# LuoweiZhou/VLP

Measured on AMD Instinct MI355X. Metric: samples/sec/node (COCO 100-region, seq64, bs64xN) fp16, higher is better.
Workload: dtype f16; 1 GPU; COCO Captions fine-tune shape: BERT-base 12L, 100 regions x 2048-d, seq_len 64 (L=167), bs 64/GPU, fwd+bwd+FP16 FusedAdam, dropout 0.1, dynamic loss scale; global_batch=64, parallelism=dp1, batch_pool=8, skipped_steps=0, rccl_ranks=1, optimizer=replicated, first_leg_packed=False

## Files before the change

### include/vlp_hip.h

```cpp
#ifndef VLP_HIP_H
#define VLP_HIP_H

#include <stdint.h>

#ifdef __cplusplus
extern "C" {
#endif

#define VLP_ABI_VERSION 5

typedef enum {
    VLP_OK = 0,
    VLP_ERR_BAD_ARG = -1,
    VLP_ERR_HIP = -2,
    VLP_ERR_WORKSPACE = -3
} vlp_status;

enum { VLP_ACT_NONE = 0, VLP_ACT_GELU = 1, VLP_ACT_RELU = 2, VLP_ACT_TANH = 3,
       VLP_ACT_GELU_SAVE_GRAD = 4  };
enum { VLP_MUL_NONE = 0, VLP_MUL_GELU_GRAD = 1, VLP_MUL_RELU_MASK = 2, VLP_MUL_PLAIN = 3  };

int vlp_version(void);
const char* vlp_last_error_string(void);
int vlp_lab_build(void);
// ... 93 lines not shown
} vlp_attn_bwd_args;
int vlp_attn_bwd(const vlp_attn_bwd_args* a, void* stream);

int vlp_mask_pack(const int64_t* mask, uint8_t* out, uint8_t* out_t, int32_t B, int32_t L, int32_t Lp, void* stream);

typedef struct {
    const void* x; int64_t ldx;
    const void* gamma; const void* beta;
    void* y; int64_t ldy;
    float* mean; float* rstd;
    int32_t M, H; float eps;
    float dropout_p; uint64_t seed; uint32_t rng_stream;
    const int32_t* row_map;
} vlp_layernorm_fwd_args;
int vlp_layernorm_fwd(const vlp_layernorm_fwd_args* a, void* stream);

typedef struct {
    const void* dy; int64_t lddy;
    const void* x; int64_t ldx;
    const void* gamma;
    const float* mean; const float* rstd;
    void* dx; int64_t lddx;
    void* dx_drop; int64_t lddxd;
    void* dgamma; void* dbeta;
    int32_t M, H; int32_t beta;
    float dy_drop_p; uint64_t dy_seed; uint32_t dy_stream;
    float out_drop_p; uint64_t out_seed; uint32_t out_stream;
    void* workspace; int64_t workspace_bytes;
    int32_t defer_reduce;
    const int32_t* row_map;
// ... 354 lines not shown
```

### vlp_amd/_lib.py

```python
import ctypes as C
import os

import torch

_HERE = os.path.dirname(os.path.abspath(__file__))
LIB_PATH = os.environ.get("VLP_HIP_LIB") or os.path.join(_HERE, "libvlp_hip.so")

ACT_NONE, ACT_GELU, ACT_RELU, ACT_TANH, ACT_GELU_SAVE_GRAD = 0, 1, 2, 3, 4
MUL_NONE, MUL_GELU_GRAD, MUL_RELU_MASK, MUL_PLAIN = 0, 1, 2, 3
ROWS_X, ROWS_MUL, ROWS_RES, ROWS_Y = 1, 2, 4, 8

vp, i64, i32, f32, u64, u32 = C.c_void_p, C.c_int64, C.c_int32, C.c_float, C.c_uint64, C.c_uint32


class GemmNtArgs(C.Structure):
    _fields_ = [("X", vp), ("ldx", i64), ("W", vp), ("ldw", i64), ("Y", vp), ("ldy", i64), ("bias", vp),
                ("residual", vp), ("ldr", i64), ("preact", vp), ("ldp", i64), ("mul_src", vp), ("ldm", i64),
                ("M", i32), ("N", i32), ("K", i32), ("act", i32), ("mul_mode", i32), ("alpha", f32),
                ("dropout_p", f32), ("seed", u64), ("rng_stream", u32), ("variant", i32), ("row_map", vp)]


class GemmTnArgs(C.Structure):
    _fields_ = [("A", vp), ("lda", i64), ("B", vp), ("ldb", i64), ("C", vp), ("ldc", i64),
                ("M", i32), ("N", i32), ("K", i32), ("beta", i32), ("workspace", vp), ("workspace_bytes", i64),
# ... 197 lines not shown
    "vlp_logsoftmax_topk": (C.c_int, [vp, i64, i32, i32, i32, vp, i32, i32, vp, vp, vp]),
    "vlp_beam_select": (C.c_int, [C.POINTER(BeamSelectArgs), vp]),
    "vlp_ngram_candidates": (C.c_int, [vp, vp, i32, i32, i32, i32, vp, i32, vp, i64, vp, vp]),
    "vlp_logsoftmax_topk_list": (C.c_int, [vp, i64, i32, i32, i32, vp, i64, vp, i32, i32, vp, vp, vp]),
    "vlp_kv_gather": (C.c_int, [vp, i64, vp, i64, vp, i32, i32, i32, i32, vp]),
    "vlp_embed_bwd_workspace_floats": (C.c_int64, [i32, i32, i32, i32]),
    "vlp_mask_build": (C.c_int, [vp, vp, vp, vp, vp, i32, i32, i32, vp, i32, vp]),
    "vlp_vis_pe_prep": (C.c_int, [C.POINTER(VisPePrepArgs), vp]),
    "vlp_sample_rows": (C.c_int, [vp, i64, i32, i32, C.c_uint64, C.c_uint32, vp, i64, vp, i64, vp]),
    "vlp_sample_rows_rep": (C.c_int, [vp, i64, i32, i32, i32, vp, C.c_uint64, C.c_uint32, vp, i64, vp, i64, vp, i64, vp]),
    "vlp_sample_rows_filtered": (C.c_int, [vp, i64, i32, i32, i32, vp, C.c_uint64, C.c_uint32, C.c_float, i32, C.c_float, vp, i64, vp, i64, vp, i64,
                                           vp, vp, vp]),
    "vlp_argmax_rows": (C.c_int, [vp, i64, i32, i32, vp, i64, vp, i64, vp]),
    "vlp_mask_pack": (C.c_int, [vp, vp, vp, i32, i32, i32, vp]),
    "vlp_layernorm_fwd": (C.c_int, [C.POINTER(LayerNormFwdArgs), vp]),
    "vlp_layernorm_bwd_workspace_bytes": (i64, [i32]),
    "vlp_layernorm_bwd": (C.c_int, [C.POINTER(LayerNormBwdArgs), vp]),
    "vlp_layernorm_bwd_rows": (C.c_int, [C.POINTER(LayerNormBwdArgs), vp, i32, i32, vp]),
    "vlp_layernorm_bwd_reduce_batched": (C.c_int, [vp, vp, i32, i32, i32, i32, vp]),
    "vlp_embed_fwd": (C.c_int, [C.POINTER(EmbedFwdArgs), vp]),
    "vlp_embed_bwd": (C.c_int, [C.POINTER(EmbedBwdArgs), vp]),
    "vlp_embed_bwd_pos": (C.c_int, [C.POINTER(EmbedBwdPosArgs), vp]),
    "vlp_scst_layout": (C.c_int, [C.POINTER(ScstLayoutArgs), vp]),
    "vlp_token_logprob_fwd": (C.c_int, [C.POINTER(TokenLogprobFwdArgs), vp]),
    "vlp_token_logprob_bwd": (C.c_int, [C.POINTER(TokenLogprobBwdArgs), vp]),
    "vlp_token_policy_fwd": (C.c_int, [C.POINTER(TokenPolicyFwdArgs), vp]),
    "vlp_token_policy_bwd": (C.c_int, [C.POINTER(TokenPolicyBwdArgs), vp]),
    "vlp_region_mask_build": (C.c_int, [vp, i32, i32, i32, vp, vp]),
    "vlp_pretext_fwd": (C.c_int, [C.POINTER(PretextFwdArgs), vp]),
    "vlp_pretext_bwd": (C.c_int, [C.POINTER(PretextBwdArgs), vp]),
# ... 138 lines not shown
                      ptr(preact), (ldp if ldp is not None else (preact.stride(0) if preact is not None else 0)),
                      ptr(mul_src), (ldm if ldm is not None else (mul_src.stride(0) if mul_src is not None else 0)),
                      M, N, K, act, mul_mode, alpha, dropout_p, seed, rng_stream, variant, ptr(row_map))


def gemm_nt(x, w, y, M, N, K, ldx=None, ldw=None, ldy=None, bias=None, residual=None, ldr=None, preact=None, ldp=None,
            mul_src=None, ldm=None, act=ACT_NONE, mul_mode=MUL_NONE, alpha=1.0, dropout_p=0.0, seed=0, rng_stream=0,
            variant=0, row_map=None):
    _req_cuda(x, w, y, row_map)
    a = _gemm_nt_args(x, w, y, M, N, K, ldx, ldw, ldy, bias, residual, ldr, preact, ldp, mul_src, ldm, act, mul_mode, alpha, dropout_p, seed,
                      rng_stream, variant, row_map)
    _check(load().vlp_gemm_nt(C.byref(a), stream_ptr()))


def gemm_nt_rows(x, w, y, live, flags, M, N, K, ldx=None, ldw=None, ldy=None, bias=None, residual=None, ldr=None, mul_src=None, ldm=None,
                 mul_mode=MUL_NONE, alpha=1.0, dropout_p=0.0, seed=0, rng_stream=0, variant=0, row_map=None):
    _req_cuda(x, w, y, live, row_map)
    a = _gemm_nt_args(x, w, y, M, N, K, ldx, ldw, ldy, bias, residual, ldr, None, None, mul_src, ldm, ACT_NONE, mul_mode, alpha, dropout_p, seed,
                      rng_stream, variant, row_map)
    _check(load().vlp_gemm_nt_rows(C.byref(a), ptr(live), flags, stream_ptr()))


def gemm_nt_resolved_variant():
    return int(load().vlp_gemm_nt_resolved_variant())


def gemm_nt_splitk_workspace_bytes(M, N, splits):
    return int(load().vlp_gemm_nt_splitk_workspace_bytes(M, N, splits))


def gemm_nt_splitk(x, w, y, M, N, K, splits, workspace, ldx=None, ldw=None, ldy=None, bias=None, residual=None, ldr=None, preact=None, ldp=None,
                   mul_src=None, ldm=None, act=ACT_NONE, mul_mode=MUL_NONE, alpha=1.0, dropout_p=0.0, seed=0, rng_stream=0):
    _req_cuda(x, w, y, workspace)
# ... 200 lines not shown
    _check(load().vlp_sample_rows_filtered(ptr(logits), ld, rows, V, rep, ptr(seed_cell), int(seed_add) & 0xFFFFFFFFFFFFFFFF, rng_stream,
                                           float(temperature), int(top_k), float(top_p), ptr(ids), ids.stride(0), ptr(ids2),
                                           ids2.stride(0) if ids2 is not None else 0, ptr(logp), logp.stride(0), ptr(cutoff), ptr(kept), stream_ptr()))


def mask_pack(mask_i64, out_u8, B, L, Lp, out_t=None):
    _req_cuda(mask_i64, out_u8, out_t)
    _check(load().vlp_mask_pack(ptr(mask_i64), ptr(out_u8), ptr(out_t), B, L, Lp, stream_ptr()))


def layernorm_fwd(x, gamma, beta, y, M, H, mean=None, rstd=None, eps=1e-5, dropout_p=0.0, seed=0, rng_stream=0, ldx=None, ldy=None, row_map=None):
    _req_cuda(x, gamma, beta, y, row_map)
    a = LayerNormFwdArgs(ptr(x), ldx if ldx is not None else x.stride(0), ptr(gamma), ptr(beta), ptr(y),
                         ldy if ldy is not None else y.stride(0), ptr(mean), ptr(rstd), M, H, eps, dropout_p, seed, rng_stream, ptr(row_map))
    _check(load().vlp_layernorm_fwd(C.byref(a), stream_ptr()))


def layernorm_bwd_workspace_bytes(H):
    return int(load().vlp_layernorm_bwd_workspace_bytes(H))


def layernorm_bwd(dy, x, gamma, mean, rstd, dx, dgamma, dbeta, M, H, workspace, beta=0, dx_drop=None,
                  dy_drop=(0.0, 0, 0), out_drop=(0.0, 0, 0), defer_reduce=False, row_map=None):
    _req_cuda(dy, x, gamma, mean, rstd, dx, dgamma, dbeta, workspace, row_map)
    a = LayerNormBwdArgs(ptr(dy), dy.stride(0), ptr(x), x.stride(0), ptr(gamma), ptr(mean), ptr(rstd), ptr(dx), dx.stride(0),
                         ptr(dx_drop), dx_drop.stride(0) if dx_drop is not None else 0, ptr(dgamma), ptr(dbeta), M, H, beta,
                         dy_drop[0], dy_drop[1], dy_drop[2], out_drop[0], out_drop[1], out_drop[2],
                         ptr(workspace), _nbytes(workspace), 1 if defer_reduce else 0, ptr(row_map))
    _check(load().vlp_layernorm_bwd(C.byref(a), stream_ptr()))

# ... 411 lines not shown
```

### vlp_amd/csrc/gemm_nt.hip

```cpp
#include "common.h"
#include "gemm_nt.h"
#include "gemm_nt_epilogue.h"

#define BM 128
#define BK 64


#ifdef VLP_NT_DEBUG
__device__ unsigned long long g_nt_trace[4096 * 4];
#define NT_TRACE(slot) do { if (wid == 0 && lane == 0 && blockIdx.x < 4096) g_nt_trace[blockIdx.x * 4 + (slot)] = wall_clock64(); } while (0)
extern "C" int vlp_debug_read_nt_trace(void* dst, int64_t bytes) { return (int)hipMemcpyFromSymbol(dst, HIP_SYMBOL(g_nt_trace), bytes); }
#else
#define NT_TRACE(slot) do { } while (0)
#endif
DEVFN int swz_x(int r) { return r & 7; }
DEVFN int swz_w(int r) { return (((r >> 4) & 3) << 1) | ((r >> 1) & 1); }

template <int VARIANT, int BM_T, int BN_T, bool SG, int NSR, int EPI, bool ROWS>
DEVFN void gemm_nt_body(const GemmNtParams& p, const int32_t* __restrict__ live, int live_flags) {
    extern __shared__ __attribute__((aligned(16))) char smem_raw[];
    f16* smem = reinterpret_cast<f16*>(smem_raw);
    constexpr int WN_ = BN_T / 64;
    constexpr int T = (BM_T / 64) * WN_ * 64;
    constexpr int RPP = T / 8;
// ... 295 lines not shown
#pragma unroll
        for (int h = 0; h < 2; ++h)
            nt_epilogue8<SG>(p, m, ncol0 + 8 * h, v + 8 * h, rkey, true);
    }
#ifdef VLP_NT_DEBUG
    NT_TRACE(2);
    asm volatile("s_waitcnt vmcnt(0)" ::: "memory");
    NT_TRACE(3);
#endif
}

template <int VARIANT, int BM_T, int BN_T, bool SG, int NSR = 0, int EPI = 0>
__global__ __launch_bounds__((BM_T / 64) * (BN_T / 64) * 64, (VARIANT == 3 ? (BN_T == 256 ? 4 : BM_T / 128) : ((VARIANT == 2 || BN_T == 256) ? 4 : 2))) void gemm_nt_kernel(GemmNtParams p) {
    gemm_nt_body<VARIANT, BM_T, BN_T, SG, NSR, EPI, false>(p, nullptr, 0);
}
__global__ __launch_bounds__(256, 1) void gemm_nt_rows_kernel(GemmNtParams p, const int32_t* __restrict__ live, int live_flags) {
    gemm_nt_body<3, 128, 128, false, 0, 0, true>(p, live, live_flags);
}

int vlp_gemm_nt_fill_params(const vlp_gemm_nt_args* a, GemmNtParams& p) {
    VLP_CHECK_ARG(a != nullptr, "vlp_gemm_nt: null args");
    VLP_CHECK_ARG(a->X && a->W && a->Y, "vlp_gemm_nt: null operand");
    VLP_CHECK_ARG(a->M > 0 && a->N > 0 && a->K > 0, "vlp_gemm_nt: bad shape M=%d N=%d K=%d", a->M, a->N, a->K);
    VLP_CHECK_ARG(a->K % BK == 0, "vlp_gemm_nt: K=%d must be a multiple of %d (pad with vlp_copy2d)", a->K, BK);
    VLP_CHECK_ARG(a->ldx % 8 == 0 && a->ldw % 8 == 0 && a->ldy % 8 == 0, "vlp_gemm_nt: leading dims must be multiples of 8 halfs");
    VLP_CHECK_ARG(a->ldx >= a->K && a->ldw >= a->K, "vlp_gemm_nt: ldx/ldw < K");
    const int n8 = (a->N + 7) / 8 * 8;
    VLP_CHECK_ARG(a->ldy >= n8, "vlp_gemm_nt: ldy=%lld < roundup8(N)=%d", (long long)a->ldy, n8);
    VLP_CHECK_ARG(((uintptr_t)a->X | (uintptr_t)a->W | (uintptr_t)a->Y) % 16 == 0, "vlp_gemm_nt: operands must be 16-byte aligned");
    if (a->residual) VLP_CHECK_ARG(a->ldr % 8 == 0 && a->ldr >= n8 && (uintptr_t)a->residual % 16 == 0, "vlp_gemm_nt: bad residual layout");
    if (a->preact) VLP_CHECK_ARG(a->ldp % 8 == 0 && a->ldp >= n8 && (uintptr_t)a->preact % 16 == 0, "vlp_gemm_nt: bad preact layout");
    if (a->mul_mode != VLP_MUL_NONE)
// ... 115 lines not shown
    }
#undef LAUNCH_RING
#undef LAUNCH_NT
#undef LAUNCH_NT_
    VLP_CHECK_LAUNCH("vlp_gemm_nt");
    return VLP_OK;
}

extern "C" int vlp_gemm_nt_rows(const vlp_gemm_nt_args* a, const int32_t* live, int32_t flags, void* stream) {
    VLP_ENTER(a ? a->X : nullptr, "vlp_gemm_nt_rows");
    GemmNtParams p;
    const int frc = vlp_gemm_nt_fill_params(a, p);
    if (frc != VLP_OK) return frc;
    VLP_CHECK_ARG(live != nullptr, "vlp_gemm_nt_rows: null row list");
    VLP_CHECK_ARG((flags & ~(VLP_ROWS_X | VLP_ROWS_MUL | VLP_ROWS_RES | VLP_ROWS_Y)) == 0, "vlp_gemm_nt_rows: bad flags %d", flags);
    VLP_CHECK_ARG(!a->preact && nt_epilogue_is_light(p) && a->act != VLP_ACT_GELU_SAVE_GRAD,
                  "vlp_gemm_nt_rows: the listed-row form carries the dgrad epilogues (bias, stored multiplier, dropout, residual) only");
    p.xcd_remap = (a->variant & 8) ? 1 : 0;
    t_last_variant = 17 | (a->variant & 8);
    const size_t smem = (size_t)4 * (128 + 128) * BK * sizeof(f16);
    VLP_ONCE_PER_DEVICE((void)hipFuncSetAttribute((const void*)gemm_nt_rows_kernel, hipFuncAttributeMaxDynamicSharedMemorySize, (int)smem));
    p.tiles_n = cdiv(a->N, 128);
    hipLaunchKernelGGL(gemm_nt_rows_kernel, dim3(cdiv(a->M, 128) * p.tiles_n), dim3(256), smem, (hipStream_t)stream, p, live, (int)flags);
    VLP_CHECK_LAUNCH("vlp_gemm_nt_rows");
    return VLP_OK;
}

extern "C" int vlp_gemm_nt_splitk(const vlp_gemm_nt_args* a, int32_t splits, void* workspace, int64_t workspace_bytes, void* stream) {
    VLP_ENTER(a ? a->X : nullptr, "vlp_gemm_nt_splitk");
    GemmNtParams p;
    const int frc = vlp_gemm_nt_fill_params(a, p);
    if (frc != VLP_OK) return frc;
    VLP_CHECK_ARG(a->act != VLP_ACT_GELU_SAVE_GRAD, "vlp_gemm_nt_splitk: VLP_ACT_GELU_SAVE_GRAD is not provided (training-shape kernels only)");
    return vlp_gemm_nt_splitk_launch(p, splits, (float*)workspace, workspace_bytes, (hipStream_t)stream);
}
```

### vlp_amd/csrc/layernorm.hip

```cpp
#include "common.h"
#include <climits>
#include <cstdlib>

#define LN_THREADS 256
#define LN_WAVES 4

DEVFN uint32_t ln_fwd_rowkey(const DropCtx& drop, const int32_t* __restrict__ row_map, int row) {
    return drop.thresh ? drop_rowkey(drop, row_map ? (uint64_t)(uint32_t)row_map[row] : (uint64_t)row) : 0u;
}
DEVFN f16 ln_fwd_out(float v, float mu, float rs, f16 gamma, f16 beta, float m) { return (f16)(((float)gamma * ((v - mu) * rs) + (float)beta) * m); }

template <int NP>
__global__ __launch_bounds__(LN_THREADS) void layernorm_fwd_kernel(
    const f16* __restrict__ x, int64_t ldx, const f16* __restrict__ gamma, const f16* __restrict__ beta,
    f16* __restrict__ y, int64_t ldy, float* __restrict__ mean, float* __restrict__ rstd, int M, int H, float eps, DropCtx drop, const int32_t* __restrict__ row_map) {
    const int lane = threadIdx.x & 63;
    const int wave = blockIdx.x * LN_WAVES + (threadIdx.x >> 6);
    const int nwaves = gridDim.x * LN_WAVES;
    const float invH = 1.f / (float)H;
    for (int row = wave; row < M; row += nwaves) {
        const f16* xr = x + (int64_t)row * ldx;
        float v[NP][4];
        float s = 0.f;
#pragma unroll
        for (int k = 0; k < NP; ++k) {
            const int c = 256 * k + 4 * lane;
            if (c < H) {
                f16x4 t = ld4(xr + c);
#pragma unroll
                for (int e = 0; e < 4; ++e) { v[k][e] = (float)t[e]; s += v[k][e]; }
            } else {
#pragma unroll
                for (int e = 0; e < 4; ++e) v[k][e] = 0.f;
            }
        }
// ... 16 lines not shown
#pragma unroll
        for (int k = 0; k < NP; ++k) {
            const int c = 256 * k + 4 * lane;
            if (c < H) {
                f16x4 gv = ld4(gamma + c), bv = ld4(beta + c), o;
                float m4[4] = {1.f, 1.f, 1.f, 1.f};
                if (drop.thresh) drop_mult4(drop, rkey, (uint32_t)c, m4);
#pragma unroll
                for (int e = 0; e < 4; ++e) o[e] = ln_fwd_out(v[k][e], mu, rs, gv[e], bv[e], m4[e]);
                st4_out<VLP_SS_LN>(yr + c, o);
            }
        }
    }
}

template <int NC>
__global__ __launch_bounds__(LN_THREADS, NC <= 3 ? 6 : 4) void layernorm_fwd_hw_kernel(
    const f16* __restrict__ x, int64_t ldx, const f16* __restrict__ gamma, const f16* __restrict__ beta,
    f16* __restrict__ y, int64_t ldy, float* __restrict__ mean, float* __restrict__ rstd, int M, int H, float eps, DropCtx drop, const int32_t* __restrict__ row_map) {
    const int lane = threadIdx.x & 63, hl = lane & 31;
    const int wave = blockIdx.x * LN_WAVES + (threadIdx.x >> 6);
    const int nwaves = gridDim.x * LN_WAVES;
    const float invH = 1.f / (float)H;
    for (int pair = wave; 2 * pair < M; pair += nwaves) {
        const int row = 2 * pair + (lane >> 5);
        const bool live = row < M;
        const f16* xr = x + (int64_t)(live ? row : M - 1) * ldx;
        f16x8 t[NC];
#pragma unroll
        for (int k = 0; k < NC; ++k) t[k] = ld8(xr + 256 * k + 8 * hl);
        float v[NC][8];
        float s = 0.f;
#pragma unroll
        for (int k = 0; k < NC; ++k)
#pragma unroll
            for (int e = 0; e < 8; ++e) { v[k][e] = (float)t[k][e]; s += v[k][e]; }
#pragma unroll
        for (int o = 16; o > 0; o >>= 1) s += __shfl_xor(s, o, 64);
        const float mu = s * invH;
        float q = 0.f;
#pragma unroll
        for (int k = 0; k < NC; ++k)
// ... 23 lines not shown
    }
}

static int env_blocks(const char* name, int dflt, int most) {
    const char* e = getenv(name);
    const int v = e ? atoi(e) : dflt;
    return v < 1 || v > most ? dflt : v;
}

static int ln_fwd_blocks(int M) {
    static const int cap = env_blocks("VLP_LN_BLOCKS", 4096, INT_MAX);
    const int blocks = cdiv(M, LN_WAVES);
    return blocks > cap ? cap : blocks;
}

extern "C" int vlp_layernorm_fwd(const vlp_layernorm_fwd_args* a, void* stream) {
    VLP_CHECK_ARG(a && a->x && a->gamma && a->beta && a->y, "vlp_layernorm_fwd: null operand");
    VLP_ENTER(a->x, "vlp_layernorm_fwd");
    VLP_CHECK_ARG(a->M > 0 && a->H > 0 && a->H % 8 == 0 && a->H <= 4096, "vlp_layernorm_fwd: H=%d must be a multiple of 8 and <= 4096", a->H);
    VLP_CHECK_ARG(a->ldx % 8 == 0 && a->ldy % 8 == 0 && a->ldx >= a->H && a->ldy >= a->H, "vlp_layernorm_fwd: leading dims");
    VLP_CHECK_ARG(((uintptr_t)a->x | (uintptr_t)a->y | (uintptr_t)a->gamma | (uintptr_t)a->beta) % 16 == 0, "vlp_layernorm_fwd: alignment");
    DropCtx d = make_drop(a->dropout_p, a->seed, a->rng_stream);
    const int blocks = ln_fwd_blocks(a->M), hblocks = ln_fwd_blocks((a->M + 1) / 2);
    hipStream_t s = (hipStream_t)stream;
#define LAUNCH_LN_FWD(KERNEL_, BLOCKS_)                                                                                        \
    hipLaunchKernelGGL(KERNEL_, dim3(BLOCKS_), dim3(LN_THREADS), 0, s, (const f16*)a->x, a->ldx, (const f16*)a->gamma,        \
                       (const f16*)a->beta, (f16*)a->y, a->ldy, a->mean, a->rstd, a->M, a->H, a->eps, d, a->row_map)
    switch (a->H) {
        case 256: LAUNCH_LN_FWD(layernorm_fwd_hw_kernel<1>, hblocks); break;
        case 512: LAUNCH_LN_FWD(layernorm_fwd_hw_kernel<2>, hblocks); break;
        case 768: LAUNCH_LN_FWD(layernorm_fwd_hw_kernel<3>, hblocks); break;
        case 1024: LAUNCH_LN_FWD(layernorm_fwd_hw_kernel<4>, hblocks); break;
        case 1536: LAUNCH_LN_FWD(layernorm_fwd_hw_kernel<6>, hblocks); break;
        case 2048: LAUNCH_LN_FWD(layernorm_fwd_hw_kernel<8>, hblocks); break;
        default:
            if (a->H <= 768) LAUNCH_LN_FWD(layernorm_fwd_kernel<3>, blocks);
            else if (a->H <= 1024) LAUNCH_LN_FWD(layernorm_fwd_kernel<4>, blocks);
            else if (a->H <= 2048) LAUNCH_LN_FWD(layernorm_fwd_kernel<8>, blocks);
            else LAUNCH_LN_FWD(layernorm_fwd_kernel<16>, blocks);
    }
#undef LAUNCH_LN_FWD
    VLP_CHECK_LAUNCH("vlp_layernorm_fwd");
    return VLP_OK;
}

#define LNB_WAVES 8
#define LNB_THREADS (64 * LNB_WAVES)
#define LNB_BLOCKS (4096 / LNB_WAVES)

template <int NP, bool EXACT, typename Sums>
DEVFN void lnb_block_partials(Sums sums, float* __restrict__ part, int H) {
    extern __shared__ float lnb_sh[];
    const int lane = threadIdx.x & 63;
    float* sg = lnb_sh + (threadIdx.x >> 6) * 2 * H;
#pragma unroll
    for (int k = 0; k < NP; ++k) {
        const int c = 256 * k + 4 * lane;
        if (EXACT || c < H) {
// ... 314 lines not shown
```

### vlp_amd/engine.py

```python
import math
import os
import weakref

import numpy as np
import torch

from . import _lib as K
from . import tuning
from .input_prep import MaskSpec, RawRegions, SparseAnswers

ALIGN = 64
NO_DECAY = ("bias", "LayerNorm.bias", "LayerNorm.weight")
PE_DIM = 1607
PE_PAD = 1664


def _ru(x, m):
    return (x + m - 1) // m * m


def is_no_decay(name):
    return any(nd in name for nd in NO_DECAY)


class VlpPerformanceWarning(UserWarning):
    """A correct but avoidably slow way of driving the engine (issued once per engine)."""


class _State(object):
    __slots__ = ("gen", "B", "L", "P", "seed", "p_drop", "ws", "batch", "has_mlm", "task_labels", "pretext", "pk", "mlm_smooth", "pos_ids", "policy")

    def __init__(self):
        self.gen = self.B = self.L = self.P = 0
        self.ws = None
        self.seed, self.p_drop = 0, (0.0, 0.0)
        self.batch = None
        self.has_mlm = False
        self.pos_ids = None
        self.pk = None
        self.pretext = None
        self.task_labels = None
        self.mlm_smooth = None
        self.policy = None


class Engine(object):
    GEMM_NT_VARIANT = None
    NT_CANDIDATES = (1, 2, 4, 5, 9, 10, 11, 12, 13, 27, 29, 73, 77, 264)
    NT_CANDIDATES_SKINNY = (1, 2, 9, 10, 11, 17)
    GEMM_TN_VARIANT = 2
    WGRAD_SIDE_STREAM = os.environ.get("VLP_WGRAD_SIDE_STREAM", "1") == "1"
    BLOCK_MASKED_REGION_KEYS = os.environ.get("VLP_BLOCK_MASKED_REGIONS", "0") == "1"
    VARLEN = {"1": True, "0": False}.get(os.environ.get("VLP_VARLEN", ""), "auto")
    TN_SPLITS = None
    TN_VARIANT_CANDIDATES = (2, 26)
    PROF_EVERY = 8
    _nt_choice = {}
    _tn_choice = {}
    _skinny_choice = {}

    def __init__(self, model):
        self._model = weakref.ref(model)
        self.packed = False
        self.gen = 0
        self.step_seed = 0
        self._warned_group_unfused = False
        self.base_seed = 0x5EED
        self.grads_dirty = False
# ... 531 lines not shown
        want_t = ws["maskt"] if train or torch.is_grad_enabled() else None
        pt = None
        if vis_masked_pos is not None and vis_masked_pos.numel() > 0:
            Pm = vis_masked_pos.shape[1]
            pt = self._pretext_workspace(ws, B, Pm)
            st_vmp = vis_masked_pos.to(torch.long).contiguous()
            K.region_mask_build(st_vmp, pt["rmask"], B, Pm, Nv)
        self._pretext_on = pt is not None
        img, prep_pe = self._region_inputs(ws, vis_feats, vis_pe)
        st = _State()
        st.gen, st.B, st.L, st.P, st.ws, st.has_mlm = self.gen, B, L, P, ws, P > 0
        st.seed, st.p_drop, st.pos_ids = seed, (p, pa), position_ids
        st.batch = (img, input_ids.contiguous(), token_type_ids.contiguous(), masked_pos)
        st.pk = (ro, rm, M) if ro is not None else None
        st.pretext = (pt, st_vmp) if pt is not None else None

        def prep_mask(am):
            if mask_spec:
                am.check(B, L)
                K.mask_build(am.second_st, am.second_end, am.is_s2s, ws["maskb"], B, L, ws["Lp"], out_t=want_t,
                             region_mask=pt["rmask"] if (pt is not None and self.BLOCK_MASKED_REGION_KEYS) else None, Nv=Nv)
            else:
                if am is None:
                    am = torch.ones(B, L, dtype=torch.long, device=input_ids.device)
                if am.dim() == 2:
                    am = am[:, None, :].expand(B, L, L)
                am = am.to(torch.long).contiguous()
                K.mask_pack(am, ws["maskb"], B, L, ws["Lp"], out_t=want_t)

        self._shadow_ev = None
        pe_ev = mask_ev = None
        if (train or torch.is_grad_enabled()) and self.WGRAD_SIDE_STREAM:
            side = self._side_stream()
            side.wait_stream(torch.cuda.current_stream())
            with torch.cuda.stream(side):
                prep_pe()
                pe_ev = torch.cuda.Event()
                pe_ev.record(side)
                prep_mask(attention_mask)
                mask_ev = torch.cuda.Event()
                mask_ev.record(side)
                if self._params_done is not None:
                    side.wait_event(self._params_done)
                if self._param_works is not None:
                    for w in self._param_works.values():
                        if w is not None:
                            w.wait()
                self._refresh_shadows()
                self._shadow_ev = torch.cuda.Event()
                self._shadow_ev.record(side)
        else:
            prep_mask(attention_mask)
            prep_pe()

        self.wait_params("nodecay")
        self.wait_params(len(self.buckets) - 1)
        self.wait_params(len(self.buckets) - 2)
        self._nt(img, self.P("vis_embed.0.weight"), ws["h1"], Mv, 2048, 2048, bias=self.P("vis_embed.0.bias"), act=K.ACT_RELU)
        self._nt(ws["h1"], self.P("vis_embed.2.weight"), ws["vis_h"], Mv, H, 2048, bias=self.P("vis_embed.2.bias"), act=K.ACT_RELU,
                 dropout_p=p, seed=seed, rng_stream=1001)
        if pe_ev is not None:
            torch.cuda.current_stream().wait_event(pe_ev)
        self._nt(ws["vpe_in"], ws["wpe_pad"], ws["vispe_h"], Mv, H, PE_PAD, bias=self.P("vis_pe_embed.0.bias"), act=K.ACT_RELU,
                 dropout_p=p, seed=seed, rng_stream=1002)
        E = "bert.embeddings."
        K.embed_fwd(st.batch[1], st.batch[2], self.P(E + "word_embeddings.weight"), self.P(E + "position_embeddings.weight"),
                    self.P(E + "token_type_embeddings.weight"), ws["vis_h"], ws["vispe_h"], ws["emb_pre"], B, L, Nv, H,
                    position_ids=position_ids, region_mask=pt["rmask"] if pt is not None else None, row_map=rm, rows=M if rm is not None else 0)
        K.layernorm_fwd(ws["emb_pre"], self.P(E + "LayerNorm.weight"), self.P(E + "LayerNorm.bias"), ws["x0"], M, H, ws["stat0"][0], ws["stat0"][1],
                        dropout_p=p, seed=seed, rng_stream=1000, row_map=rm)
        x = ws["x0"]
        scale = 1.0 / math.sqrt(H // A)
        for i in range(NL):
            Ln = "bert.encoder.layer.%d." % i
            a = ws["layers"][i]
            self.wait_params(NL - i)
            self._nt(x, self.P(Ln + "attention.self.query.weight"), a["qkv"], M, 3 * H, H, bias=self.P(Ln + "attention.self.query.bias"))
            if i == 0 and mask_ev is not None:
                torch.cuda.current_stream().wait_event(mask_ev)
            K.attn_fwd(a["qkv"], ws["maskb"], a["ctx"], a["lse"], B, L, A, scale, dropout_p=pa, seed=seed, rng_stream=16 * i + 1, row_off=ro)
            self._nt(a["ctx"], self.P(Ln + "attention.output.dense.weight"), a["pre1"], M, H, H, bias=self.P(Ln + "attention.output.dense.bias"),
                     residual=x, dropout_p=p, seed=seed, rng_stream=16 * i + 2, row_map=rm)
            K.layernorm_fwd(a["pre1"], self.P(Ln + "attention.output.LayerNorm.weight"), self.P(Ln + "attention.output.LayerNorm.bias"),
                            a["x1"], M, H, a["st1"][0], a["st1"][1])
            self._nt(a["x1"], self.P(Ln + "intermediate.dense.weight"), a["g"], M, I, H, bias=self.P(Ln + "intermediate.dense.bias"),
                     preact=a["z"], act=K.ACT_GELU_SAVE_GRAD)
            self._nt(a["g"], self.P(Ln + "output.dense.weight"), a["pre2"], M, H, I, bias=self.P(Ln + "output.dense.bias"),
                     residual=a["x1"], dropout_p=p, seed=seed, rng_stream=16 * i + 3, row_map=rm)
            K.layernorm_fwd(a["pre2"], self.P(Ln + "output.LayerNorm.weight"), self.P(Ln + "output.LayerNorm.bias"), a["x2"], M, H,
                            a["st2"][0], a["st2"][1])
            x = a["x2"]
        self.wait_params(0)
        if P > 0:
            C = "cls.predictions."
            R = B * P
# ... 46 lines not shown
                raise RuntimeError("SparseAnswers must live on the GPU (there is no CPU path)")
            st.task_labels = SparseAnswers(ans_labels.idx.contiguous(), ans_labels.score.contiguous(), ans_labels.verified_for)
            K.bce_sparse_loss_fwd(ws["vq_logits"], ws["NAp"], st.task_labels.idx, st.task_labels.score, st.B, NA, ws["loss"])
            return ws["loss"][0:1]
        st.task_labels = ans_labels.to(torch.float32).contiguous()
        K.bce_loss_fwd(ws["vq_logits"], ws["NAp"], st.task_labels, st.task_labels.stride(0), st.B, NA, ws["loss"])
        return ws["loss"][0:1]

    def mlm_logits(self, st):
        V = self._model().config.vocab_size
        return st.ws["logits"][:, :V].view(st.B, st.P, V)

    def vqa_logits(self, st):
        return st.ws["vq_logits"][:, :self._model().num_answers]

    def sequence_output(self, st):
        cfg = self._model().config
        x = st.ws["layers"][cfg.num_hidden_layers - 1]["x2"]
        if st.pk is not None:
            dense = torch.zeros(st.B * st.L, cfg.hidden_size, device=x.device, dtype=x.dtype)
            K.rows_unpack(x, st.pk[1], st.pk[2], dense, cfg.hidden_size)
            x = dense
        return x.view(st.B, st.L, cfg.hidden_size)

    def _decode_workspace(self, B, T0, Lcap, Kb=1, group=False):
        key = ("dec", B, T0, Lcap, Kb) + (("group",) if group else ())
        ws = self._ws.get(key)
        if ws is not None:
            return ws
        model = self._model()
        cfg = model.config
# ... 499 lines not shown
            else:
                K.gemm_tn_grouped_rows(listed)
                self._tn(*qkv[:6], ws, beta, bias=qkv[7])
            self._bucket_done(cfg.num_hidden_layers - i)
            if use_side:
                ev = torch.cuda.Event()
                ev.record(side)
                self._side_done[i & 1] = ev
        on_side(last_wgrad)
        self._nt(dqkv, s["qkvT"], dx, M, H, 3 * H, residual=dpre1)

    def backward(self, st, gscale, task, g_pretext=None, g_rows=None, h_rows=None):
        if st.gen != self.gen:
            raise RuntimeError("vlp_amd: the activations of this forward were overwritten by a later forward "
                               "(one in-flight forward per model; run backward before the next forward)")
        model = self._model()
        cfg = model.config
        H, I, A, NL, Nv, V = cfg.hidden_size, cfg.intermediate_size, cfg.num_attention_heads, cfg.num_hidden_layers, model.len_vis_input, cfg.vocab_size
        B, L, P, ws, seed = st.B, st.L, st.P, st.ws, st.seed
        p, pa = st.p_drop
        M, Mv = B * L, B * Nv
        ro = rm = None
        if st.pk is not None:
            ro, rm, M = st.pk
        beta = 1 if self.grads_dirty else 0
        if beta and self.shard_plan is not None:
            raise RuntimeError("vlp_amd: VLP_DDP_MODE=sharded keeps only this rank's chunk of the reduced gradient, so gradients cannot be "
                               "accumulated over several backward passes (--gradient_accumulation_steps > 1); use allreduce or rs_ag")
        img, input_ids, token_type_ids, masked_pos = st.batch
        self.wait_params()
# ... 16 lines not shown
        side = self._side_stream() if use_side else None

        def on_side(fn):
            if not use_side:
                fn()
                return
            side.wait_stream(main)
            with torch.cuda.stream(side):
                fn()

        if use_side:
            self._side_busy = True
        head_wgrads = []

        live = live_ready = None
        if (task != "vqa2" and task != "logprob" and st.has_mlm and P > 0 and st.pretext is None
                and os.environ.get("VLP_LAST_LAYER_LIVE", "1") != "0"):
            live, Rl = ws["lv_rows"], B * P

            def live_prologue():
                K.live_rows_build(masked_pos.contiguous(), B, P, L, live, ws["lv_n"], row_off=ro)
                ws["dctx"][:M].zero_()
                ws["dyset"][(NL - 1) & 1]["dpre1"][:M].zero_()
            on_side(live_prologue)
            if use_side:
                live_ready = torch.cuda.Event()
                live_ready.record(side)
        self._live_n = ws["lv_n"] if live is not None else None

        if task == "vqa2":
            NA, NAp = model.num_answers, ws["NAp"]
            if isinstance(st.task_labels, SparseAnswers):
                K.bce_sparse_loss_bwd(ws["vq_logits"], NAp, st.task_labels.idx, st.task_labels.score, B, NA, gscale, ws["vq_dlogits"], NAp)
            else:
                K.bce_loss_bwd(ws["vq_logits"], NAp, st.task_labels, st.task_labels.stride(0), B, NA, gscale, ws["vq_dlogits"], NAp)
            self._tn(ws["vq_dlogits"], ws["vq_a1"], self.G("ans_classifier.2.weight"), B, NA, 2 * H, ws, beta, bias=self.G("ans_classifier.2.bias"))
# ... 179 lines not shown
```

Baseline: 6706 samples/s.

## Compute last encoder layer's post-attention forward only at masked rows

```diff
diff --git a/include/vlp_hip.h b/include/vlp_hip.h
--- a/include/vlp_hip.h
+++ b/include/vlp_hip.h
@@ -131,6 +131,7 @@
     const int32_t* row_map;
 } vlp_layernorm_fwd_args;
 int vlp_layernorm_fwd(const vlp_layernorm_fwd_args* a, void* stream);
+int vlp_layernorm_fwd_rows(const vlp_layernorm_fwd_args* a, const int32_t* live, void* stream);
 
 typedef struct {
     const void* dy; int64_t lddy;
diff --git a/vlp_amd/_lib.py b/vlp_amd/_lib.py
--- a/vlp_amd/_lib.py
+++ b/vlp_amd/_lib.py
@@ -235,6 +235,7 @@
     "vlp_argmax_rows": (C.c_int, [vp, i64, i32, i32, vp, i64, vp, i64, vp]),
     "vlp_mask_pack": (C.c_int, [vp, vp, vp, i32, i32, i32, vp]),
     "vlp_layernorm_fwd": (C.c_int, [C.POINTER(LayerNormFwdArgs), vp]),
+    "vlp_layernorm_fwd_rows": (C.c_int, [C.POINTER(LayerNormFwdArgs), vp, vp]),
     "vlp_layernorm_bwd_workspace_bytes": (i64, [i32]),
     "vlp_layernorm_bwd": (C.c_int, [C.POINTER(LayerNormBwdArgs), vp]),
     "vlp_layernorm_bwd_rows": (C.c_int, [C.POINTER(LayerNormBwdArgs), vp, i32, i32, vp]),
@@ -403,9 +404,9 @@
 
 
 def gemm_nt_rows(x, w, y, live, flags, M, N, K, ldx=None, ldw=None, ldy=None, bias=None, residual=None, ldr=None, mul_src=None, ldm=None,
-                 mul_mode=MUL_NONE, alpha=1.0, dropout_p=0.0, seed=0, rng_stream=0, variant=0, row_map=None):
-    _req_cuda(x, w, y, live, row_map)
-    a = _gemm_nt_args(x, w, y, M, N, K, ldx, ldw, ldy, bias, residual, ldr, None, None, mul_src, ldm, ACT_NONE, mul_mode, alpha, dropout_p, seed,
+                 mul_mode=MUL_NONE, alpha=1.0, dropout_p=0.0, seed=0, rng_stream=0, variant=0, row_map=None, preact=None, ldp=None, act=ACT_NONE):
+    _req_cuda(x, w, y, live, row_map, preact)
+    a = _gemm_nt_args(x, w, y, M, N, K, ldx, ldw, ldy, bias, residual, ldr, preact, ldp, mul_src, ldm, act, mul_mode, alpha, dropout_p, seed,
                       rng_stream, variant, row_map)
     _check(load().vlp_gemm_nt_rows(C.byref(a), ptr(live), flags, stream_ptr()))
 
@@ -636,6 +637,13 @@
     a = LayerNormFwdArgs(ptr(x), ldx if ldx is not None else x.stride(0), ptr(gamma), ptr(beta), ptr(y),
                          ldy if ldy is not None else y.stride(0), ptr(mean), ptr(rstd), M, H, eps, dropout_p, seed, rng_stream, ptr(row_map))
     _check(load().vlp_layernorm_fwd(C.byref(a), stream_ptr()))
+
+
+def layernorm_fwd_rows(x, gamma, beta, y, live, M, H, mean=None, rstd=None, eps=1e-5, dropout_p=0.0, seed=0, rng_stream=0, row_map=None):
+    _req_cuda(x, gamma, beta, y, live, row_map)
+    a = LayerNormFwdArgs(ptr(x), x.stride(0), ptr(gamma), ptr(beta), ptr(y), y.stride(0), ptr(mean), ptr(rstd), M, H, eps, dropout_p, seed, rng_stream,
+                         ptr(row_map))
+    _check(load().vlp_layernorm_fwd_rows(C.byref(a), ptr(live), stream_ptr()))
 
 
 def layernorm_bwd_workspace_bytes(H):
diff --git a/vlp_amd/csrc/gemm_nt.hip b/vlp_amd/csrc/gemm_nt.hip
--- a/vlp_amd/csrc/gemm_nt.hip
+++ b/vlp_amd/csrc/gemm_nt.hip
@@ -333,8 +333,9 @@
 __global__ __launch_bounds__((BM_T / 64) * (BN_T / 64) * 64, (VARIANT == 3 ? (BN_T == 256 ? 4 : BM_T / 128) : ((VARIANT == 2 || BN_T == 256) ? 4 : 2))) void gemm_nt_kernel(GemmNtParams p) {
     gemm_nt_body<VARIANT, BM_T, BN_T, SG, NSR, EPI, false>(p, nullptr, 0);
 }
+template <bool SG>
 __global__ __launch_bounds__(256, 1) void gemm_nt_rows_kernel(GemmNtParams p, const int32_t* __restrict__ live, int live_flags) {
-    gemm_nt_body<3, 128, 128, false, 0, 0, true>(p, live, live_flags);
+    gemm_nt_body<3, 128, 128, SG, 0, 0, true>(p, live, live_flags);
 }
 
 int vlp_gemm_nt_fill_params(const vlp_gemm_nt_args* a, GemmNtParams& p) {
@@ -480,14 +481,26 @@
     if (frc != VLP_OK) return frc;
     VLP_CHECK_ARG(live != nullptr, "vlp_gemm_nt_rows: null row list");
     VLP_CHECK_ARG((flags & ~(VLP_ROWS_X | VLP_ROWS_MUL | VLP_ROWS_RES | VLP_ROWS_Y)) == 0, "vlp_gemm_nt_rows: bad flags %d", flags);
-    VLP_CHECK_ARG(!a->preact && nt_epilogue_is_light(p) && a->act != VLP_ACT_GELU_SAVE_GRAD,
-                  "vlp_gemm_nt_rows: the listed-row form carries the dgrad epilogues (bias, stored multiplier, dropout, residual) only");
+    const bool sg = a->act == VLP_ACT_GELU_SAVE_GRAD;
+    if (sg) {
+        VLP_CHECK_ARG(!a->residual && a->mul_mode == VLP_MUL_NONE && a->dropout_p == 0.f,
+                      "vlp_gemm_nt_rows: VLP_ACT_GELU_SAVE_GRAD fuses bias + gelu + derivative only (no residual / multiplier / dropout)");
+    } else {
+        VLP_CHECK_ARG(!a->preact && nt_epilogue_is_light(p),
+                      "vlp_gemm_nt_rows: the listed-row form carries bias, stored multiplier, dropout and residual, or the save-grad GeLU, only");
+    }
     p.xcd_remap = (a->variant & 8) ? 1 : 0;
     t_last_variant = 17 | (a->variant & 8);
     const size_t smem = (size_t)4 * (128 + 128) * BK * sizeof(f16);
-    VLP_ONCE_PER_DEVICE((void)hipFuncSetAttribute((const void*)gemm_nt_rows_kernel, hipFuncAttributeMaxDynamicSharedMemorySize, (int)smem));
     p.tiles_n = cdiv(a->N, 128);
-    hipLaunchKernelGGL(gemm_nt_rows_kernel, dim3(cdiv(a->M, 128) * p.tiles_n), dim3(256), smem, (hipStream_t)stream, p, live, (int)flags);
+    const dim3 grid(cdiv(a->M, 128) * p.tiles_n);
+    if (sg) {
+        VLP_ONCE_PER_DEVICE((void)hipFuncSetAttribute((const void*)gemm_nt_rows_kernel<true>, hipFuncAttributeMaxDynamicSharedMemorySize, (int)smem));
+        hipLaunchKernelGGL(gemm_nt_rows_kernel<true>, grid, dim3(256), smem, (hipStream_t)stream, p, live, (int)flags);
+    } else {
+        VLP_ONCE_PER_DEVICE((void)hipFuncSetAttribute((const void*)gemm_nt_rows_kernel<false>, hipFuncAttributeMaxDynamicSharedMemorySize, (int)smem));
+        hipLaunchKernelGGL(gemm_nt_rows_kernel<false>, grid, dim3(256), smem, (hipStream_t)stream, p, live, (int)flags);
+    }
     VLP_CHECK_LAUNCH("vlp_gemm_nt_rows");
     return VLP_OK;
 }
diff --git a/vlp_amd/csrc/layernorm.hip b/vlp_amd/csrc/layernorm.hip
--- a/vlp_amd/csrc/layernorm.hip
+++ b/vlp_amd/csrc/layernorm.hip
@@ -10,15 +10,18 @@
 }
 DEVFN f16 ln_fwd_out(float v, float mu, float rs, f16 gamma, f16 beta, float m) { return (f16)(((float)gamma * ((v - mu) * rs) + (float)beta) * m); }
 
-template <int NP>
+template <int NP, bool LIST = false>
 __global__ __launch_bounds__(LN_THREADS) void layernorm_fwd_kernel(
     const f16* __restrict__ x, int64_t ldx, const f16* __restrict__ gamma, const f16* __restrict__ beta,
-    f16* __restrict__ y, int64_t ldy, float* __restrict__ mean, float* __restrict__ rstd, int M, int H, float eps, DropCtx drop, const int32_t* __restrict__ row_map) {
+    f16* __restrict__ y, int64_t ldy, float* __restrict__ mean, float* __restrict__ rstd, int M, int H, float eps, DropCtx drop, const int32_t* __restrict__ row_map,
+    const int32_t* __restrict__ list) {
     const int lane = threadIdx.x & 63;
     const int wave = blockIdx.x * LN_WAVES + (threadIdx.x >> 6);
     const int nwaves = gridDim.x * LN_WAVES;
     const float invH = 1.f / (float)H;
-    for (int row = wave; row < M; row += nwaves) {
+    for (int m = wave; m < M; m += nwaves) {
+        const int row = LIST ? list[m] : m;
+        if (LIST && row < 0) continue;
         const f16* xr = x + (int64_t)row * ldx;
         float v[NP][4];
         float s = 0.f;
@@ -65,18 +68,20 @@
     }
 }
 
-template <int NC>
+template <int NC, bool LIST = false>
 __global__ __launch_bounds__(LN_THREADS, NC <= 3 ? 6 : 4) void layernorm_fwd_hw_kernel(
     const f16* __restrict__ x, int64_t ldx, const f16* __restrict__ gamma, const f16* __restrict__ beta,
-    f16* __restrict__ y, int64_t ldy, float* __restrict__ mean, float* __restrict__ rstd, int M, int H, float eps, DropCtx drop, const int32_t* __restrict__ row_map) {
+    f16* __restrict__ y, int64_t ldy, float* __restrict__ mean, float* __restrict__ rstd, int M, int H, float eps, DropCtx drop, const int32_t* __restrict__ row_map,
+    const int32_t* __restrict__ list) {
     const int lane = threadIdx.x & 63, hl = lane & 31;
     const int wave = blockIdx.x * LN_WAVES + (threadIdx.x >> 6);
     const int nwaves = gridDim.x * LN_WAVES;
     const float invH = 1.f / (float)H;
     for (int pair = wave; 2 * pair < M; pair += nwaves) {
-        const int row = 2 * pair + (lane >> 5);
-        const bool live = row < M;
-        const f16* xr = x + (int64_t)(live ? row : M - 1) * ldx;
+        const int m = 2 * pair + (lane >> 5);
+        const int row = LIST ? (m < M ? list[m] : -1) : m;
+        const bool live = LIST ? row >= 0 : row < M;
+        const f16* xr = x + (int64_t)(live ? row : (LIST ? 0 : M - 1)) * ldx;
         f16x8 t[NC];
 #pragma unroll
         for (int k = 0; k < NC; ++k) t[k] = ld8(xr + 256 * k + 8 * hl);
@@ -130,9 +135,7 @@
     return blocks > cap ? cap : blocks;
 }
 
-extern "C" int vlp_layernorm_fwd(const vlp_layernorm_fwd_args* a, void* stream) {
-    VLP_CHECK_ARG(a && a->x && a->gamma && a->beta && a->y, "vlp_layernorm_fwd: null operand");
-    VLP_ENTER(a->x, "vlp_layernorm_fwd");
+static int ln_fwd_launch(const vlp_layernorm_fwd_args* a, const int32_t* list, void* stream) {
     VLP_CHECK_ARG(a->M > 0 && a->H > 0 && a->H % 8 == 0 && a->H <= 4096, "vlp_layernorm_fwd: H=%d must be a multiple of 8 and <= 4096", a->H);
     VLP_CHECK_ARG(a->ldx % 8 == 0 && a->ldy % 8 == 0 && a->ldx >= a->H && a->ldy >= a->H, "vlp_layernorm_fwd: leading dims");
     VLP_CHECK_ARG(((uintptr_t)a->x | (uintptr_t)a->y | (uintptr_t)a->gamma | (uintptr_t)a->beta) % 16 == 0, "vlp_layernorm_fwd: alignment");
@@ -141,7 +144,22 @@
     hipStream_t s = (hipStream_t)stream;
 #define LAUNCH_LN_FWD(KERNEL_, BLOCKS_)                                                                                        \
     hipLaunchKernelGGL(KERNEL_, dim3(BLOCKS_), dim3(LN_THREADS), 0, s, (const f16*)a->x, a->ldx, (const f16*)a->gamma,        \
-                       (const f16*)a->beta, (f16*)a->y, a->ldy, a->mean, a->rstd, a->M, a->H, a->eps, d, a->row_map)
+                       (const f16*)a->beta, (f16*)a->y, a->ldy, a->mean, a->rstd, a->M, a->H, a->eps, d, a->row_map, list)
+    if (list) {
+        switch (a->H) {
+            case 256: LAUNCH_LN_FWD((layernorm_fwd_hw_kernel<1, true>), hblocks); break;
+            case 512: LAUNCH_LN_FWD((layernorm_fwd_hw_kernel<2, true>), hblocks); break;
+            case 768: LAUNCH_LN_FWD((layernorm_fwd_hw_kernel<3, true>), hblocks); break;
+            case 1024: LAUNCH_LN_FWD((layernorm_fwd_hw_kernel<4, true>), hblocks); break;
+            case 1536: LAUNCH_LN_FWD((layernorm_fwd_hw_kernel<6, true>), hblocks); break;
+            case 2048: LAUNCH_LN_FWD((layernorm_fwd_hw_kernel<8, true>), hblocks); break;
+            default:
+                if (a->H <= 768) LAUNCH_LN_FWD((layernorm_fwd_kernel<3, true>), blocks);
+                else if (a->H <= 1024) LAUNCH_LN_FWD((layernorm_fwd_kernel<4, true>), blocks);
+                else if (a->H <= 2048) LAUNCH_LN_FWD((layernorm_fwd_kernel<8, true>), blocks);
+                else LAUNCH_LN_FWD((layernorm_fwd_kernel<16, true>), blocks);
+        }
+    } else
     switch (a->H) {
         case 256: LAUNCH_LN_FWD(layernorm_fwd_hw_kernel<1>, hblocks); break;
         case 512: LAUNCH_LN_FWD(layernorm_fwd_hw_kernel<2>, hblocks); break;
@@ -158,6 +176,18 @@
 #undef LAUNCH_LN_FWD
     VLP_CHECK_LAUNCH("vlp_layernorm_fwd");
     return VLP_OK;
+}
+
+extern "C" int vlp_layernorm_fwd(const vlp_layernorm_fwd_args* a, void* stream) {
+    VLP_CHECK_ARG(a && a->x && a->gamma && a->beta && a->y, "vlp_layernorm_fwd: null operand");
+    VLP_ENTER(a->x, "vlp_layernorm_fwd");
+    return ln_fwd_launch(a, nullptr, stream);
+}
+
+extern "C" int vlp_layernorm_fwd_rows(const vlp_layernorm_fwd_args* a, const int32_t* live, void* stream) {
+    VLP_CHECK_ARG(a && a->x && a->gamma && a->beta && a->y && live, "vlp_layernorm_fwd_rows: null operand");
+    VLP_ENTER(a->x, "vlp_layernorm_fwd_rows");
+    return ln_fwd_launch(a, live, stream);
 }
 
 #define LNB_WAVES 8
diff --git a/vlp_amd/engine.py b/vlp_amd/engine.py
--- a/vlp_amd/engine.py
+++ b/vlp_amd/engine.py
@@ -28,7 +28,7 @@
 
 
 class _State(object):
-    __slots__ = ("gen", "B", "L", "P", "seed", "p_drop", "ws", "batch", "has_mlm", "task_labels", "pretext", "pk", "mlm_smooth", "pos_ids", "policy")
+    __slots__ = ("gen", "B", "L", "P", "seed", "p_drop", "ws", "batch", "has_mlm", "task_labels", "pretext", "pk", "mlm_smooth", "pos_ids", "policy", "live_fwd")
 
     def __init__(self):
         self.gen = self.B = self.L = self.P = 0
@@ -42,6 +42,7 @@
         self.task_labels = None
         self.mlm_smooth = None
         self.policy = None
+        self.live_fwd = False
 
 
 class Engine(object):
@@ -52,6 +53,7 @@
     WGRAD_SIDE_STREAM = os.environ.get("VLP_WGRAD_SIDE_STREAM", "1") == "1"
     BLOCK_MASKED_REGION_KEYS = os.environ.get("VLP_BLOCK_MASKED_REGIONS", "0") == "1"
     VARLEN = {"1": True, "0": False}.get(os.environ.get("VLP_VARLEN", ""), "auto")
+    LIVE_FWD_MIN_ROWS = 6144
     TN_SPLITS = None
     TN_VARIANT_CANDIDATES = (2, 26)
     PROF_EVERY = 8
@@ -613,6 +615,13 @@
         st.batch = (img, input_ids.contiguous(), token_type_ids.contiguous(), masked_pos)
         st.pk = (ro, rm, M) if ro is not None else None
         st.pretext = (pt, st_vmp) if pt is not None else None
+        live_fwd = (bool(train) and P > 0 and not want_vqa and pt is None and not dense and M >= self.LIVE_FWD_MIN_ROWS
+                    and os.environ.get("VLP_LAST_LAYER_LIVE", "1") != "0")
+        st.live_fwd = live_fwd
+        live_ev = None
+
+        def live_list():
+            K.live_rows_build(masked_pos.contiguous(), B, P, L, ws["lv_rows"], ws["lv_n"], row_off=ro)
 
         def prep_mask(am):
             if mask_spec:
@@ -639,6 +648,10 @@
                 prep_mask(attention_mask)
                 mask_ev = torch.cuda.Event()
                 mask_ev.record(side)
+                if live_fwd:
+                    live_list()
+                    live_ev = torch.cuda.Event()
+                    live_ev.record(side)
                 if self._params_done is not None:
                     side.wait_event(self._params_done)
                 if self._param_works is not None:
@@ -651,6 +664,8 @@
         else:
             prep_mask(attention_mask)
             prep_pe()
+            if live_fwd:
+                live_list()
 
         self.wait_params("nodecay")
         self.wait_params(len(self.buckets) - 1)
@@ -678,6 +693,12 @@
             if i == 0 and mask_ev is not None:
                 torch.cuda.current_stream().wait_event(mask_ev)
             K.attn_fwd(a["qkv"], ws["maskb"], a["ctx"], a["lse"], B, L, A, scale, dropout_p=pa, seed=seed, rng_stream=16 * i + 1, row_off=ro)
+            if live_fwd and i == NL - 1:
+                if live_ev is not None:
+                    torch.cuda.current_stream().wait_event(live_ev)
+                self._layer_fwd_live(i, a, x, ws["lv_rows"], B * P, p, seed, rm)
+                x = a["x2"]
+                continue
             self._nt(a["ctx"], self.P(Ln + "attention.output.dense.weight"), a["pre1"], M, H, H, bias=self.P(Ln + "attention.output.dense.bias"),
                      residual=x, dropout_p=p, seed=seed, rng_stream=16 * i + 2, row_map=rm)
             K.layernorm_fwd(a["pre1"], self.P(Ln + "attention.output.LayerNorm.weight"), self.P(Ln + "attention.output.LayerNorm.bias"),
@@ -754,7 +775,26 @@
     def vqa_logits(self, st):
         return st.ws["vq_logits"][:, :self._model().num_answers]
 
+    def _layer_fwd_live(self, i, a, x, live, R, p, seed, rm):
+        cfg = self._model().config
+        H, I = cfg.hidden_size, cfg.intermediate_size
+        Ln = "bert.encoder.layer.%d." % i
+        io = K.ROWS_X | K.ROWS_Y
+        K.gemm_nt_rows(a["ctx"], self.P(Ln + "attention.output.dense.weight"), a["pre1"], live, io | K.ROWS_RES, R, H, H,
+                       bias=self.P(Ln + "attention.output.dense.bias"), residual=x, dropout_p=p, seed=seed, rng_stream=16 * i + 2, row_map=rm)
+        K.layernorm_fwd_rows(a["pre1"], self.P(Ln + "attention.output.LayerNorm.weight"), self.P(Ln + "attention.output.LayerNorm.bias"),
+                             a["x1"], live, R, H, a["st1"][0], a["st1"][1])
+        K.gemm_nt_rows(a["x1"], self.P(Ln + "intermediate.dense.weight"), a["g"], live, io, R, I, H, bias=self.P(Ln + "intermediate.dense.bias"),
+                       preact=a["z"], act=K.ACT_GELU_SAVE_GRAD)
+        K.gemm_nt_rows(a["g"], self.P(Ln + "output.dense.weight"), a["pre2"], live, io | K.ROWS_RES, R, H, I, bias=self.P(Ln + "output.dense.bias"),
+                       residual=a["x1"], dropout_p=p, seed=seed, rng_stream=16 * i + 3, row_map=rm)
+        K.layernorm_fwd_rows(a["pre2"], self.P(Ln + "output.LayerNorm.weight"), self.P(Ln + "output.LayerNorm.bias"), a["x2"], live, R, H,
+                             a["st2"][0], a["st2"][1])
+
     def sequence_output(self, st):
+        if st.live_fwd:
+            raise RuntimeError("vlp_amd: this masked-LM training forward computed the last layer's hidden states at the masked positions only; "
+                               "set VLP_LAST_LAYER_LIVE=0 to compute every row (sequence_output needs them)")
         cfg = self._model().config
         x = st.ws["layers"][cfg.num_hidden_layers - 1]["x2"]
         if st.pk is not None:
@@ -1284,6 +1324,10 @@
         if st.gen != self.gen:
             raise RuntimeError("vlp_amd: the activations of this forward were overwritten by a later forward "
                                "(one in-flight forward per model; run backward before the next forward)")
+        live_ok = task != "vqa2" and task != "logprob" and st.has_mlm and st.P > 0 and st.pretext is None
+        if st.live_fwd and not live_ok:
+            raise RuntimeError("vlp_amd: backward(task=%r) needs every row of the last layer, but this forward computed it at the masked "
+                               "positions only (a masked-LM training forward); set VLP_LAST_LAYER_LIVE=0" % (task,))
         model = self._model()
         cfg = model.config
         H, I, A, NL, Nv, V = cfg.hidden_size, cfg.intermediate_size, cfg.num_attention_heads, cfg.num_hidden_layers, model.len_vis_input, cfg.vocab_size
@@ -1330,12 +1374,12 @@
         head_wgrads = []
 
         live = live_ready = None
-        if (task != "vqa2" and task != "logprob" and st.has_mlm and P > 0 and st.pretext is None
-                and os.environ.get("VLP_LAST_LAYER_LIVE", "1") != "0"):
+        if live_ok and (st.live_fwd or os.environ.get("VLP_LAST_LAYER_LIVE", "1") != "0"):
             live, Rl = ws["lv_rows"], B * P
 
             def live_prologue():
-                K.live_rows_build(masked_pos.contiguous(), B, P, L, live, ws["lv_n"], row_off=ro)
+                if not st.live_fwd:
+                    K.live_rows_build(masked_pos.contiguous(), B, P, L, live, ws["lv_n"], row_off=ro)
                 ws["dctx"][:M].zero_()
                 ws["dyset"][(NL - 1) & 1]["dpre1"][:M].zero_()
             on_side(live_prologue)
```

Result: no change. 6753 samples/s, median of 6 (+0.7%).
